# louissmit/VBNN

Measured on AMD Instinct MI355X. Metric: VBLinear fwd+bwd samples/sec, higher is better.
Workload: dtype bf16; 1 GPU; 784-4096-4096-10 VBLinear MLP, batch 4096 per GPU, LRT, S=1; mode=lrt, global_batch=4096, parallelism=dp1, warmup_steps_run=255, backward_order=every updateGradInput, then the accGradParameters from the first layer up, launch=one stream launch per kernel

## Files before the change

### vbnn_amd/csrc/elementwise.hip

```cpp
#include "common.h"

static inline int grid_for(int64_t work_items, int per_block) {
    int64_t b = (work_items + per_block - 1) / per_block;
    if (b < 1) b = 1;
    if (b > 2048) b = 2048;
    return (int)b;
}

template <bool HW>
__global__ __launch_bounds__(256) void k_fill_normal(float* out, int64_t rows, int64_t cols, int64_t ld, uint64_t seed,
                                                     uint32_t stream, uint32_t layer, uint32_t draw, int64_t row0, float scale) {
    const int64_t quads = (cols + 3) >> 2;
    const int64_t total = rows * quads;
    for (int64_t t = (int64_t)blockIdx.x * 256 + threadIdx.x; t < total; t += (int64_t)gridDim.x * 256) {
        const int64_t r = t / quads, q = t - r * quads;
        const vbnn_f32x4 z = HW ? vbnn_normal4_hw(seed, stream, layer, draw, (uint32_t)(row0 + r), (uint32_t)q)
                                : vbnn_normal4(seed, stream, layer, draw, (uint32_t)(row0 + r), (uint32_t)q);
        float* p = out + r * ld + q * 4;
        const int valid = (int)min((int64_t)4, cols - q * 4);
        const bool vec = ((ld & 3) == 0) && (((uintptr_t)out & 15u) == 0);
        store4<float>(p, z.v[0] * scale, z.v[1] * scale, z.v[2] * scale, z.v[3] * scale, valid, vec);
    }
}

// ... 1010 lines not shown
        else hipLaunchKernelGGL(k_update_finish<bf16_t>, dim3(n_layers + pack_blocks), dim3(256), 0, ctx->stream, fa);
    }
    return vbnn_check_launch("vbnn_update");
    VBNN_API_END
}

template <typename T>
__global__ __launch_bounds__(256) void k_pack_input(const float* __restrict__ src, int64_t ld_src, int64_t N, int64_t I, T* x_s,
                                                    T* x2_s, int64_t ld_x, T* xT_s, T* x2T_s, int64_t ld_xT, int64_t rpd) {
    __shared__ float ta[64][65];
    __shared__ float tb[64][65];
    const int64_t tiles_c = (I + 63) / 64, tiles_r = (N + 63) / 64;
    const int64_t ntiles = tiles_c * tiles_r;
    const bool vec_in = ((ld_src & 3) == 0) && (((uintptr_t)src & 15u) == 0);
    const bool vec_t = (ld_xT & 3) == 0;
    for (int64_t tI = blockIdx.x; tI < ntiles; tI += gridDim.x) {
        const int64_t r0 = (tI / tiles_c) * 64, c0 = (tI % tiles_c) * 64;
#pragma unroll
        for (int k = 0; k < 4; ++k) {
            const int idx = threadIdx.x + 256 * k;
            const int rr = idx >> 4, c4 = (idx & 15) * 4;
            const int64_t r = r0 + rr, c = c0 + c4;
            float a[4] = {0.f, 0.f, 0.f, 0.f}, b[4] = {0.f, 0.f, 0.f, 0.f};
            const int valid = (r < N) ? (int)min((int64_t)4, I - c) : 0;
            if (valid > 0) {
                load4<float>(src + (rpd > 0 ? r % rpd : r) * ld_src + c, a, valid, vec_in);
#pragma unroll
                for (int e = 0; e < 4; ++e) { const float ar = Elt<T>::from(Elt<T>::to(a[e])); b[e] = ar * ar; }
                store4<T>(x_s + r * ld_x + c, a[0], a[1], a[2], a[3], valid, true);
                if (x2_s) store4<T>(x2_s + r * ld_x + c, b[0], b[1], b[2], b[3], valid, true);
            }
#pragma unroll
            for (int e = 0; e < 4; ++e) { ta[rr][c4 + e] = a[e]; tb[rr][c4 + e] = b[e]; }
        }
        if (xT_s) {
            __syncthreads();
#pragma unroll
            for (int k = 0; k < 4; ++k) {
                const int idx = threadIdx.x + 256 * k;
                const int cc = idx >> 4, r4 = (idx & 15) * 4;
                const int64_t c = c0 + cc, r = r0 + r4;
                const int valid = (c < I) ? (int)min((int64_t)4, N - r) : 0;
                if (valid > 0) {
                    store4<T>(xT_s + c * ld_xT + r, ta[r4][cc], ta[r4 + 1][cc], ta[r4 + 2][cc], ta[r4 + 3][cc], valid, vec_t);
                    if (x2T_s)
                        store4<T>(x2T_s + c * ld_xT + r, tb[r4][cc], tb[r4 + 1][cc], tb[r4 + 2][cc], tb[r4 + 3][cc], valid, vec_t);
                }
            }
            __syncthreads();
        }
    }
}

extern "C" int vbnn_pack_input(vbnn_ctx* ctx, int dtype, const float* src, int64_t ld_src, int64_t N, int64_t I, void* x_s,
                               void* x2_s, int64_t ld_x, void* xT_s, void* x2T_s, int64_t ld_xT, int64_t rows_per_draw) {
    VBNN_API_BEGIN
    VBNN_REQUIRE(ctx && src && x_s, "null argument");
    VBNN_REQUIRE(rows_per_draw >= 0, "rows_per_draw");
    VBNN_REQUIRE(N > 0 && I > 0 && ld_src >= I && ld_x >= I && ld_x % 4 == 0, "shape");
    VBNN_REQUIRE(!x2T_s || xT_s, "x2T_s needs xT_s");
    VBNN_REQUIRE(!xT_s || ld_xT >= N, "ld_xT");
    const int64_t ntiles = ((N + 63) / 64) * ((I + 63) / 64);
    const int nb = (int)(ntiles < 4096 ? ntiles : 4096);
    if (dtype == VBNN_F32)
        hipLaunchKernelGGL(k_pack_input<float>, dim3(nb), dim3(256), 0, ctx->stream, src, ld_src, N, I, (float*)x_s, (float*)x2_s,
                           ld_x, (float*)xT_s, (float*)x2T_s, ld_xT, rows_per_draw);
    else if (dtype == VBNN_BF16)
        hipLaunchKernelGGL(k_pack_input<bf16_t>, dim3(nb), dim3(256), 0, ctx->stream, src, ld_src, N, I, (bf16_t*)x_s,
                           (bf16_t*)x2_s, ld_x, (bf16_t*)xT_s, (bf16_t*)x2T_s, ld_xT, rows_per_draw);
    else { vbnn_set_error("unsupported dtype %d", dtype); return VBNN_ERR_UNSUPPORTED; }
    return vbnn_check_launch("k_pack_input");
    VBNN_API_END
}

template <bool TO_BF16>
__global__ __launch_bounds__(256) void k_cast_grads(const void* __restrict__ src, void* __restrict__ dst, int64_t n, int vec) {
    const int64_t i0 = ((int64_t)blockIdx.x * 256 + threadIdx.x) * 8;
    if (i0 >= n) return;
    if (vec && i0 + 8 <= n) {
        if constexpr (TO_BF16) {
            const f32x4 a = reinterpret_cast<const f32x4*>(static_cast<const float*>(src) + i0)[0];
            const f32x4 b = reinterpret_cast<const f32x4*>(static_cast<const float*>(src) + i0)[1];
            reinterpret_cast<bf16x8*>(static_cast<bf16_t*>(dst) + i0)[0] =
                bf16x8{(bf16_t)a[0], (bf16_t)a[1], (bf16_t)a[2], (bf16_t)a[3], (bf16_t)b[0], (bf16_t)b[1], (bf16_t)b[2], (bf16_t)b[3]};
        } else {
            const bf16x8 v = reinterpret_cast<const bf16x8*>(static_cast<const bf16_t*>(src) + i0)[0];
            reinterpret_cast<f32x4*>(static_cast<float*>(dst) + i0)[0] = f32x4{(float)v[0], (float)v[1], (float)v[2], (float)v[3]};
            reinterpret_cast<f32x4*>(static_cast<float*>(dst) + i0)[1] = f32x4{(float)v[4], (float)v[5], (float)v[6], (float)v[7]};
        }
    } else {
        for (int64_t i = i0; i < n && i < i0 + 8; ++i) {
            if constexpr (TO_BF16) static_cast<bf16_t*>(dst)[i] = (bf16_t)static_cast<const float*>(src)[i];
            else static_cast<float*>(dst)[i] = (float)static_cast<const bf16_t*>(src)[i];
        }
    }
}

extern "C" int vbnn_cast_grads(vbnn_ctx* ctx, int to_bf16, const void* src, void* dst, int64_t n) {
    VBNN_API_BEGIN
    VBNN_REQUIRE(ctx && src && dst && n > 0, "argument");
    const int vec = (((uintptr_t)src | (uintptr_t)dst) & 15u) == 0;
    const unsigned nb = (unsigned)((n + 2047) / 2048);
    if (to_bf16) hipLaunchKernelGGL(k_cast_grads<true>, dim3(nb), dim3(256), 0, ctx->stream, src, dst, n, vec);
    else hipLaunchKernelGGL(k_cast_grads<false>, dim3(nb), dim3(256), 0, ctx->stream, src, dst, n, vec);
    return vbnn_check_launch("k_cast_grads");
    VBNN_API_END
}

struct StatsCombineArgs { double* stats[8]; int n_layers, world; const double* parts; };
__global__ void k_stats_combine(StatsCombineArgs a) {
    const int l = threadIdx.x;
    if (l >= a.n_layers) return;
    double s0 = 0.0, s1 = 0.0, w = 0.0;
    for (int r = 0; r < a.world; ++r) {
// ... 47 lines not shown
```

### vbnn_amd/csrc/head.hip

```cpp
#include "common.h"
#include "gemm_v1.h"

constexpr int HEAD_CMAX = 16;
constexpr int HEAD_FW = 8;

template <typename T> struct Vec8;
template <> struct Vec8<bf16_t> {
    typedef bf16x8 raw_t;
    static __device__ __forceinline__ raw_t load_raw(const bf16_t* p) { return *reinterpret_cast<const bf16x8*>(p); }
    static __device__ __forceinline__ void cvt(const raw_t& t, float (&v)[8]) {
#pragma unroll
        for (int e = 0; e < 8; ++e) v[e] = (float)t[e];
    }
    static __device__ __forceinline__ raw_t load_guarded(const bf16_t* p, int valid) {
        raw_t t;
#pragma unroll
        for (int e = 0; e < 8; ++e) t[e] = e < valid ? p[e] : (bf16_t)0.f;
        return t;
    }
    static __device__ __forceinline__ void load(const bf16_t* p, float (&v)[8]) {
        const bf16x8 t = *reinterpret_cast<const bf16x8*>(p);
#pragma unroll
        for (int e = 0; e < 8; ++e) v[e] = (float)t[e];
    }
// ... 28 lines not shown
        *reinterpret_cast<f32x4*>(p) = f32x4{v[0], v[1], v[2], v[3]};
        *reinterpret_cast<f32x4*>(p + 4) = f32x4{v[4], v[5], v[6], v[7]};
    }
};

__device__ __forceinline__ float head_sum_partials(const float* src, int64_t stride, int R) {
    float tot = 0.f;
    int r = 0;
    for (; r + 8 <= R; r += 8) {
        float p[8];
#pragma unroll
        for (int u = 0; u < 8; ++u) p[u] = vbnn_load_wt(src + (int64_t)(r + u) * stride);
#pragma unroll
        for (int u = 0; u < 8; ++u) tot += p[u];
    }
    if (r < R) {
        float p[8];
#pragma unroll
        for (int u = 0; u < 8; ++u) p[u] = (r + u < R) ? vbnn_load_wt(src + (int64_t)(r + u) * stride) : 0.f;
#pragma unroll
        for (int u = 0; u < 8; ++u) if (r + u < R) tot += p[u];
    }
    return tot;
}

__device__ __forceinline__ void head_row_max(const float (&v)[4], int q, float& mx, int& arg) {
    mx = -INFINITY; arg = 0x7fffffff;
#pragma unroll
    for (int j = 0; j < 4; ++j)
        if (v[j] > mx) { mx = v[j]; arg = 4 * q + j; }
#pragma unroll
    for (int off = 16; off <= 32; off <<= 1) {
        const float om = __shfl_xor(mx, off, 64);
        const int oa = __shfl_xor(arg, off, 64);
        if (om > mx || (om == mx && oa < arg)) { mx = om; arg = oa; }
    }
}

__device__ __forceinline__ void head_log_softmax(f32x4 s, int q, int C, const float* __restrict__ bias, float (&lg)[4], int& arg, float& lse) {
#pragma unroll
    for (int j = 0; j < 4; ++j) {
        const int c = 4 * q + j;
        lg[j] = (c < C) ? s[j] + (bias ? bias[c] : 0.f) : -INFINITY;
    }
    float mx;
    head_row_max(lg, q, mx, arg);
    float se = 0.f;
#pragma unroll
    for (int j = 0; j < 4; ++j) if (4 * q + j < C) se += expf(lg[j] - mx);
    se += __shfl_xor(se, 16, 64);
    se += __shfl_xor(se, 32, 64);
    lse = mx + logf(se);
}

__device__ __forceinline__ void head_rows_from_logits(f32x4 s, int lane, int64_t n0, int64_t N, int C, const float* __restrict__ bias,
                                                      const int32_t* __restrict__ target, int64_t rpd, float inv_n, float* out, float* g_logits,
                                                      float* logits, double* part_loss, int32_t* part_corr) {
    const int q = lane >> 4, c16 = lane & 15;
    const int64_t n = n0 + c16;
    const bool row_ok = n < N;
    float lg[4];
    int arg;
    float lse;
    head_log_softmax(s, q, C, bias, lg, arg, lse);
    const int t = row_ok ? min(max(target[rpd > 0 ? n % rpd : n], 0), C - 1) : 0;
    double loss_acc = 0.0;
#pragma unroll
    for (int j = 0; j < 4; ++j) {
        const int c = 4 * q + j;
        if (row_ok && c < C) {
            const float o = lg[j] - lse;
            if (logits) logits[n * C + c] = lg[j];
            if (out) out[n * C + c] = o;
            g_logits[n * C + c] = (expf(o) - (c == t ? 1.0f : 0.0f)) * inv_n;
            if (c == t) loss_acc -= (double)o * (double)inv_n;
        }
    }
    int corr = (row_ok && q == 0 && arg == t) ? 1 : 0;
#pragma unroll
    for (int off = 32; off > 0; off >>= 1) { loss_acc += __shfl_xor(loss_acc, off, 64); corr += __shfl_xor(corr, off, 64); }
    if (lane == 0) { vbnn_store_wt(&part_loss[blockIdx.x], loss_acc); vbnn_store_wt(&part_corr[blockIdx.x], (int32_t)corr); }
}

template <int NT>
__device__ __forceinline__ void head_sum_loss_partials(unsigned* counter, const double* part_loss, const int32_t* part_corr, double* loss_sum,
                                                       int32_t* correct, int accumulate, double* red_l, int* red_c, int* last) {
    if (!vbnn_last_arriver(counter, gridDim.x, last)) return;
    const int lane = threadIdx.x & 63, wave = threadIdx.x >> 6;
    double ls = 0.0;
    int cs = 0;
    for (int b = (int)threadIdx.x; b < (int)gridDim.x; b += NT) { ls += vbnn_load_wt(&part_loss[b]); cs += vbnn_load_wt(&part_corr[b]); }
#pragma unroll
    for (int off = 32; off > 0; off >>= 1) { ls += __shfl_xor(ls, off, 64); cs += __shfl_xor(cs, off, 64); }
    if (lane == 0) { red_l[wave] = ls; red_c[wave] = cs; }
    __syncthreads();
    if (threadIdx.x == 0) {
        double lt = 0.0;
        int ct = 0;
#pragma unroll
        for (int w = 0; w < NT / 64; ++w) { lt += red_l[w]; ct += red_c[w]; }
        if (loss_sum) loss_sum[0] = (accumulate ? loss_sum[0] : 0.0) + lt;
        if (correct) correct[0] = (accumulate ? correct[0] : 0) + ct;
    }
}

template <typename T>
__device__ __forceinline__ f32x4 head_logits_wave(const T* __restrict__ hp, const T* __restrict__ wp, int64_t k_lo, int64_t k_hi) {
// ... 458 lines not shown
        }
    }
    auto put = [&](float* p, float v) { if (fin_tickets) vbnn_store_wt(p, v); else *p = v; };
    if (partial_w) {
        const int64_t i = c0 + 16 * wave + c16;
        if (i < H) {
#pragma unroll
            for (int j = 0; j < 4; ++j)
                if (4 * q + j < C) put(&partial_w[((int64_t)blockIdx.y * C + 4 * q + j) * H + i], accw[j]);
            if (partial_bp && q == 0) put(&partial_bp[(int64_t)blockIdx.y * H + i], accp[0]);
        }
    }
    if (partial_b && blockIdx.x == 0) {
        __syncthreads();
        float* red = reinterpret_cast<float*>(&th[0][0]);
        red[tid] = accb;
        __syncthreads();
        if (tid < C) {
            float tot = 0.f;
#pragma unroll
            for (int rg = 0; rg < 16; ++rg) tot += red[rg * 16 + tid];
            put(&partial_b[(int64_t)blockIdx.y * C + tid], tot);
        }
    }
    if (!fin_tickets) return;
    __shared__ int fin_last;
    if (!vbnn_last_arriver(fin_tickets + blockIdx.x, gridDim.y, &fin_last)) return;
    const int R = (int)gridDim.y;
    const int64_t nw = (int64_t)C * H;
    for (int k = tid; k < C * 64 + 64; k += 256) {
        const bool is_w = k < C * 64;
        const int64_t i = c0 + (is_w ? k & 63 : k - C * 64);
        if (i >= H) continue;
        float* dst = is_w ? (fin_gw ? fin_gw + (int64_t)(k >> 6) * H + i : nullptr) : (fin_gbp ? fin_gbp + i : nullptr);
        if (!dst) continue;
        const float* src = is_w ? partial_w + (int64_t)(k >> 6) * H + i : partial_bp + i;
        const int64_t stride = is_w ? nw : H;
        const float tot = head_sum_partials(src, stride, R);
        *dst = (fin_accumulate ? *dst : 0.f) + tot;
    }
    if (blockIdx.x == 0 && tid < C && fin_gb) {
        const float tot = head_sum_partials(partial_b + tid, C, R);
        fin_gb[tid] = (fin_accumulate ? fin_gb[tid] : 0.f) + tot;
    }
}

typedef __bf16 hb_bf16x2 __attribute__((ext_vector_type(2)));
__device__ __forceinline__ float hb_dot2(unsigned a, unsigned b, float c) {
    return __builtin_amdgcn_fdot2_f32_bf16(__builtin_bit_cast(hb_bf16x2, a), __builtin_bit_cast(hb_bf16x2, b), c, false);
}
__device__ __forceinline__ unsigned hb_bf16_bits(float v) {
    return (unsigned)__builtin_bit_cast(unsigned short, (bf16_t)v);
}
template <int U, int HEAD_SW >
__global__ __launch_bounds__(64 * HEAD_SW) void k_head_backward_stream(
    const bf16_t* __restrict__ h, int64_t ld_h, const bf16_t* __restrict__ w3, int64_t ld_w, const float* __restrict__ g, int64_t N,
    int64_t H, int C, int relu_mask, const bf16_t* __restrict__ r_prev, int64_t ld_r, bf16_t* __restrict__ g_prev,
    bf16_t* __restrict__ gv_prev, int64_t ld_gp, int rows_per_chunk, float* __restrict__ partial_w ,
    float* __restrict__ partial_b , float* __restrict__ partial_bp ,
    unsigned* fin_tickets , int fin_accumulate, float* fin_gw, float* fin_gb, float* fin_gbp) {
    static_assert(U == 2 || U == 4, "2 or 4 hidden units per lane");
    constexpr int CP = 12, NP = CP / 2, UW = U / 2;
    typedef float accv __attribute__((ext_vector_type(U)));
    typedef unsigned rawv __attribute__((ext_vector_type(UW)));
    __shared__ accv red[4][HEAD_SW][64];
    const int tid = threadIdx.x, lane = tid & 63, wave = tid >> 6;
    const int64_t cb0 = (int64_t)blockIdx.x * (64 * U);
    const int64_t c0 = cb0 + U * lane;
    const int64_t n_lo = (int64_t)blockIdx.y * rows_per_chunk, n_hi = min(N, n_lo + rows_per_chunk);
    unsigned wp[NP][U];
    {
        unsigned wr[CP][UW];
#pragma unroll
        for (int c = 0; c < CP; ++c) {
            rawv t = 0u;
            if (c < C) t = *reinterpret_cast<const rawv*>(w3 + (int64_t)c * ld_w + c0);
#pragma unroll
            for (int k = 0; k < UW; ++k) wr[c][k] = ((const unsigned*)&t)[k];
        }
#pragma unroll
        for (int p = 0; p < NP; ++p)
#pragma unroll
            for (int e = 0; e < U; ++e) {
                const unsigned lo = (wr[2 * p][e >> 1] >> (16 * (e & 1))) & 0xffffu, hi = (wr[2 * p + 1][e >> 1] >> (16 * (e & 1))) & 0xffffu;
                wp[p][e] = lo | (hi << 16);
            }
    }
    float accw[CP][U], accb[U], accg = 0.f;
#pragma unroll
    for (int e = 0; e < U; ++e) accb[e] = 0.f;
#pragma unroll
    for (int c = 0; c < CP; ++c)
#pragma unroll
        for (int e = 0; e < U; ++e) accw[c][e] = 0.f;
    const int gcls = lane < CP ? lane : lane - CP;
    const bool gl_on = lane < 2 * CP && gcls < C;
    const bool has_r = r_prev != nullptr;
    const unsigned lo_h = (unsigned)(U * lane);
    auto ldrow = [&](int64_t n, rawv& hv, rawv& rv) {
        hv = *reinterpret_cast<const rawv*>(h + (n * ld_h + cb0) + lo_h);
        rv = 0u;
        if (has_r) rv = *reinterpret_cast<const rawv*>(r_prev + (n * ld_r + cb0) + lo_h);
    };
    auto ldg = [&](int64_t n) { return gl_on ? g[(n + (lane >= CP ? 1 : 0)) * C + gcls] : 0.f; };
    auto word = [](const rawv& v, int k) { return ((const unsigned*)&v)[k]; };
    int64_t n = n_lo + 2 * wave;
    rawv h0 = 0u, h1 = 0u, r0 = 0u, r1 = 0u;
    float gv = 0.f;
    if (n < n_hi) { ldrow(n, h0, r0); ldrow(n + 1, h1, r1); gv = ldg(n); }
    for (; n < n_hi; n += 2 * HEAD_SW) {
        const rawv hh[2] = {h0, h1}, rr[2] = {r0, r1};
        const float cg = gv;
        const int64_t nn = n + 2 * HEAD_SW;
        if (nn < n_hi) { ldrow(nn, h0, r0); ldrow(nn + 1, h1, r1); gv = ldg(nn); }
        accg += cg;
        const unsigned gb = hb_bf16_bits(cg);
        unsigned g0[CP], g1[CP];
#pragma unroll
        for (int c = 0; c < CP; ++c) { g0[c] = __builtin_amdgcn_readlane(gb, c); g1[c] = __builtin_amdgcn_readlane(gb, CP + c); }
#pragma unroll
        for (int row = 0; row < 2; ++row) {
            const unsigned* gs = row ? g1 : g0;
            float gx[U];
#pragma unroll
            for (int e = 0; e < U; ++e) gx[e] = 0.f;
#pragma unroll
            for (int p = 0; p < NP; ++p) {
                const unsigned gp2 = gs[2 * p] | (gs[2 * p + 1] << 16);
#pragma unroll
                for (int e = 0; e < U; ++e) gx[e] = hb_dot2(gp2, wp[p][e], gx[e]);
            }
            unsigned gbits[U], vbits[U];
#pragma unroll
            for (int e = 0; e < U; ++e) {
                const unsigned hw = word(hh[row], e >> 1), rw = word(rr[row], e >> 1);
                const float hv = __builtin_bit_cast(float, (e & 1) ? (hw & 0xffff0000u) : (hw << 16));
                const float rv = __builtin_bit_cast(float, (e & 1) ? (rw & 0xffff0000u) : (rw << 16));
                const float gp = (relu_mask && !(hv > 0.f)) ? 0.f : gx[e];
                gbits[e] = hb_bf16_bits(gp);
                vbits[e] = hb_bf16_bits(has_r ? gp * rv : 0.f);
                accb[e] += __builtin_bit_cast(float, gbits[e] << 16);
            }
            const int64_t ro = (n + row) * ld_gp + cb0;
            rawv og, ov;
#pragma unroll
            for (int k = 0; k < UW; ++k) { ((unsigned*)&og)[k] = gbits[2 * k] | (gbits[2 * k + 1] << 16); ((unsigned*)&ov)[k] = vbits[2 * k] | (vbits[2 * k + 1] << 16); }
            *reinterpret_cast<rawv*>(g_prev + ro + lo_h) = og;
            if (gv_prev) *reinterpret_cast<rawv*>(gv_prev + ro + lo_h) = ov;
        }
        unsigned hp[U];
#pragma unroll
        for (int e = 0; e < U; ++e) {
            const unsigned a = word(hh[0], e >> 1), b = word(hh[1], e >> 1);
            hp[e] = (e & 1) ? ((a >> 16) | (b & 0xffff0000u)) : ((a & 0xffffu) | (b << 16));
        }
#pragma unroll
        for (int c = 0; c < CP; ++c) {
            const unsigned gr2 = g0[c] | (g1[c] << 16);
#pragma unroll
            for (int e = 0; e < U; ++e) accw[c][e] = hb_dot2(gr2, hp[e], accw[c][e]);
        }
    }
    const int64_t chunk = blockIdx.y;
    auto put = [&](float* p, const accv& t) {
        if (!fin_tickets) { *reinterpret_cast<accv*>(p) = t; return; }
#pragma unroll
        for (int e = 0; e < U; e += 2) vbnn_store_wt2(p + e, t[e], t[e + 1]);
    };
    auto meet = [&](const accv (&q)[4], int nq, auto&& emit) {
        __syncthreads();
#pragma unroll
        for (int k = 0; k < 4; ++k)
            if (k < nq) red[k][wave][lane] = q[k];
        __syncthreads();
        if (wave < nq) {
            accv t = red[wave][0][lane];
#pragma unroll
            for (int w = 1; w < HEAD_SW; ++w) t += red[wave][w][lane];
            emit(wave, t);
        }
    };
#pragma unroll
    for (int c4 = 0; c4 < CP; c4 += 4) {
        accv q[4];
#pragma unroll
        for (int k = 0; k < 4; ++k)
#pragma unroll
            for (int e = 0; e < U; ++e) q[k][e] = accw[c4 + k][e];
        meet(q, 4, [&](int k, accv t) {
            if (partial_w && c4 + k < C) put(partial_w + ((chunk * C + c4 + k) * H + c0), t);
        });
    }
    {
        accv q[4];
#pragma unroll
        for (int k = 0; k < 4; ++k)
#pragma unroll
            for (int e = 0; e < U; ++e) q[k][e] = (k == 0) ? accb[e] : ((k == 1 && e == 0) ? accg : 0.f);
        meet(q, 2, [&](int k, accv t) {
            const float odd = __shfl(t[0], (lane + CP) & 63, 64);
            if (k == 0) { if (partial_bp) put(partial_bp + (chunk * H + c0), t); }
            else if (partial_b && blockIdx.x == 0 && lane < CP && lane < C) {
                if (fin_tickets) vbnn_store_wt(&partial_b[chunk * C + lane], t[0] + odd); else partial_b[chunk * C + lane] = t[0] + odd;
            }
        });
    }
    if (!fin_tickets) return;
    __shared__ int fin_last;
    if (!vbnn_last_arriver(fin_tickets + blockIdx.x, gridDim.y, &fin_last)) return;
    const int R = (int)gridDim.y;
    const int64_t nw = (int64_t)C * H;
    constexpr int CB = 64 * U;
    for (int k = tid; k < C * CB + CB; k += 64 * HEAD_SW) {
// ... 276 lines not shown
                                       int64_t N, int64_t C, float inv_n, float* logits, float* out, float* g_logits, int accumulate,
                                       double* loss_sum_dev, int32_t* correct_dev, int64_t rows_per_draw) {
    VBNN_API_BEGIN
    VBNN_REQUIRE(ctx && slots && target && g_logits, "null argument");
    VBNN_REQUIRE(rows_per_draw >= 0, "rows_per_draw");
    VBNN_REQUIRE(N > 0 && C > 0 && C <= HEAD_CMAX && n_slots > 0 && n_slots < (1 << 20), "shape (C <= 16)");
    VBNN_REQUIRE(((uintptr_t)slots & 15u) == 0, "slots must be 16-byte aligned");
    const unsigned nb = (unsigned)((N + 15) / 16);
    VBNN_REQUIRE((size_t)nb * 2 <= ctx->scratch_doubles, "minibatch too large for the reduction scratch");
    double* part_loss = ctx->scratch;
    int32_t* part_corr = reinterpret_cast<int32_t*>(ctx->scratch + nb);
    hipLaunchKernelGGL(k_head_from_slots, dim3(nb), dim3(64), 0, ctx->stream, slots, (int)n_slots, bias, target, N, (int)C, inv_n, out,
                       g_logits, logits, loss_sum_dev, correct_dev, accumulate, part_loss, part_corr, ctx->counters + VBNN_CNT_HEAD_FWD,
                       rows_per_draw);
    return vbnn_check_launch("k_head_from_slots");
    VBNN_API_END
}

extern "C" int vbnn_head_predict(vbnn_ctx* ctx, int dtype, const vbnn_predict_args* a) {
    VBNN_API_BEGIN
    VBNN_REQUIRE(ctx && a && a->h && a->w3, "null argument");
    VBNN_REQUIRE(a->R > 0 && a->H > 0 && a->C > 0 && a->C <= HEAD_CMAX, "shape (C <= 16)");
    VBNN_REQUIRE(a->S >= 1 && a->S < (1ll << 24), "draws S >= 1");
    VBNN_REQUIRE(a->form == VBNN_PREDICT_STACKED || a->form == VBNN_PREDICT_ACCUMULATE, "form");
    VBNN_REQUIRE(a->ld_h % VBNN_KPAD == 0 && a->ld_w % VBNN_KPAD == 0 && a->ld_h >= a->H && a->ld_w >= a->H, "h and w3 must be packed operands");
    VBNN_REQUIRE((((uintptr_t)a->h | (uintptr_t)a->w3) & 15u) == 0, "operands must be 16-byte aligned");
    VBNN_REQUIRE(!a->totals || a->target, "totals need targets");
    const bool stacked = a->form == VBNN_PREDICT_STACKED;
    const int draws = stacked ? (int)a->S : 1;
    const int first = stacked ? 1 : (a->first ? 1 : 0), fin = stacked ? 1 : (a->final ? 1 : 0);
    VBNN_REQUIRE(a->state || (first && fin), "the accumulating form keeps its running state in `state`");
    VBNN_REQUIRE(a->R * draws < (1ll << 40), "rows");
    const unsigned nb = (unsigned)((a->R + 15) / 16);
    VBNN_REQUIRE((size_t)nb * 4 <= ctx->scratch_doubles, "minibatch too large for the reduction scratch");
    double* part = ctx->scratch;
    unsigned* ticket = ctx->counters + VBNN_CNT_PREDICT;
    if (dtype == VBNN_F32) {
        const int64_t Hp = (a->H + 15) / 16 * 16;
        hipLaunchKernelGGL(k_head_predict<float>, dim3(nb), dim3(64 * HEAD_FW), 0, ctx->stream, (const float*)a->h, a->ld_h,
                           (const float*)a->w3, a->ld_w, a->bias, a->target, a->R, Hp, (int)a->C, draws, (int)a->S, first, fin,
                           a->state, a->probs, a->log_probs, a->entropy, a->expected_entropy, a->mutual_info, a->pred, a->totals,
                           part, ticket);
    } else if (dtype == VBNN_BF16) {
        const int64_t Hp = (a->H + 31) / 32 * 32;
        hipLaunchKernelGGL(k_head_predict<bf16_t>, dim3(nb), dim3(64 * HEAD_FW), 0, ctx->stream, (const bf16_t*)a->h, a->ld_h,
                           (const bf16_t*)a->w3, a->ld_w, a->bias, a->target, a->R, Hp, (int)a->C, draws, (int)a->S, first, fin,
                           a->state, a->probs, a->log_probs, a->entropy, a->expected_entropy, a->mutual_info, a->pred, a->totals,
                           part, ticket);
    } else { vbnn_set_error("unsupported dtype %d", dtype); return VBNN_ERR_UNSUPPORTED; }
    return vbnn_check_launch("k_head_predict");
    VBNN_API_END
}

static int g_head_inline_finish = 1;
template <typename T>
static int head_backward_t(vbnn_ctx* ctx, const T* h, int64_t ld_h, const T* w3, int64_t ld_w, const float* g_logits, int64_t N,
                           int64_t H, int64_t C, int accumulate, float* gradWeight, float* gradBias, float* gradBias_prev,
                           int relu_mask, const void* r_prev_any, int64_t ld_r_prev, int r_prev_packed, T* g_prev, T* gv_prev,
                           int64_t ld_gp, T* gT_prev, T* gvT_prev, int64_t ld_gpT) {
    const float* r_prev = r_prev_packed ? nullptr : (const float*)r_prev_any;
    const T* r_prev_t = r_prev_packed ? (const T*)r_prev_any : nullptr;
    const bool sums = gradWeight || gradBias || gradBias_prev;
    if (!sums && !g_prev && !gT_prev) return VBNN_OK;
    static const bool env_read = [] { const char* e = getenv("VBNN_HEAD_INLINE_FINISH"); if (e && e[0] == '0') g_head_inline_finish = 0; return true; }();
    (void)env_read;
    const int64_t tiles_c = (H + 63) / 64, tiles_r = (N + 63) / 64;
    const int64_t per_chunk = C * H + C + H;
    const int64_t cap = (int64_t)(ctx->scratch_doubles * 2) / per_chunk;
    VBNN_REQUIRE(!sums || cap >= 1, "hidden size too large for the reduction scratch");
    int64_t R = (2 * (int64_t)vbnn_cu_count() + tiles_c - 1) / tiles_c;
    static const int env_blocks = [] { const char* e = getenv("VBNN_HEAD_BLOCKS"); return e ? atoi(e) : 0; }();
    if (env_blocks > 0) R = (env_blocks + tiles_c - 1) / tiles_c;
    if (R > tiles_r) R = tiles_r;
    if (sums && R > cap) R = cap;
    if (R < 1) R = 1;
    VBNN_REQUIRE(R <= 65535, "too many row chunks");
    const int rows_per_chunk = (int)((tiles_r + R - 1) / R) * 64;
    R = (N + rows_per_chunk - 1) / rows_per_chunk;
    float* partial_w = reinterpret_cast<float*>(ctx->scratch);
    float* partial_b = partial_w + R * C * H;
    float* partial_bp = partial_b + R * C;
    const bool vec = (ld_h % 8 == 0) && (!r_prev_any || ld_r_prev % 8 == 0) && (!g_prev || ld_gp % 8 == 0) &&
                     (!(gT_prev || gvT_prev) || ld_gpT % 8 == 0) &&
                     ((((uintptr_t)h | (uintptr_t)r_prev_any | (uintptr_t)g_prev | (uintptr_t)gv_prev | (uintptr_t)gT_prev |
                        (uintptr_t)gvT_prev) & 15u) == 0);
    const dim3 grid((unsigned)tiles_c, (unsigned)R);
    float* pw = (gradWeight || gradBias_prev) ? partial_w : nullptr;
    float* pb = gradBias ? partial_b : nullptr;
    float* pbp = gradBias_prev ? partial_bp : nullptr;
    const bool full = vec && (H % 64 == 0) && (N % 64 == 0) && N * ld_h < (1ll << 31) && N * ld_gp < (1ll << 31) &&
                      H * ld_gpT < (1ll << 31) && (!r_prev_any || N * ld_r_prev < (1ll << 31));
    const bool inline_fin = sums && tiles_c * R <= vbnn_cu_count() && tiles_c <= VBNN_CNT_TILES_MAX && g_head_inline_finish;
    unsigned* ft = inline_fin ? ctx->counters + VBNN_CNT_TILES : nullptr;
    static const bool env_stream = [] { const char* e = getenv("VBNN_HEAD_STREAM"); return !(e && e[0] == '0'); }();
    if constexpr (sizeof(T) == 2) {
        const bool want = g_head_stream == 1 || (g_head_stream == -1 && env_stream && !inline_fin);
        if (want && full && C <= 12 && !r_prev && g_prev && !gT_prev && !gvT_prev && H % 128 == 0 && N % 32 == 0) {
            constexpr int SU = 2, SWV = 16;
            if (H % (64 * SU) == 0 && N % (2 * SWV) == 0) {
            const int64_t cb = H / (64 * SU);
            int64_t Rs = ((int64_t)vbnn_cu_count() + cb - 1) / cb;
            if (Rs < 1) Rs = 1;
            if (sums && Rs > cap) Rs = cap;
            const int rpc = (int)(((N + Rs - 1) / Rs + 2 * SWV - 1) / (2 * SWV) * (2 * SWV));
            Rs = (N + rpc - 1) / rpc;
            float* spw = reinterpret_cast<float*>(ctx->scratch);
            float* spb = spw + Rs * C * H;
            float* spbp = spb + Rs * C;
#define VBNN_HS_LAUNCH(UU, WW) hipLaunchKernelGGL((k_head_backward_stream<UU, WW>), dim3((unsigned)cb, (unsigned)Rs), dim3(64 * WW), 0, ctx->stream, (const bf16_t*)h, ld_h, \
                               (const bf16_t*)w3, ld_w, g_logits, N, H, (int)C, relu_mask, (const bf16_t*)r_prev_t, ld_r_prev, (bf16_t*)g_prev,  \
                               (bf16_t*)gv_prev, ld_gp, rpc, (gradWeight || gradBias_prev) ? spw : nullptr, gradBias ? spb : nullptr,         \
                               gradBias_prev ? spbp : nullptr, sft, accumulate, gradWeight, gradBias, gradBias_prev)
            unsigned* sft = (sums && g_head_inline_finish && cb <= VBNN_CNT_TILES_MAX) ? ctx->counters + VBNN_CNT_TILES : nullptr;
            VBNN_HS_LAUNCH(SU, SWV);
#undef VBNN_HS_LAUNCH
            if (sums && !sft) {
                const int64_t outs = C * H + (gradBias_prev ? H : 0);
                hipLaunchKernelGGL(k_head_backward_finish, dim3((unsigned)((outs + 255) / 256)), dim3(256), 0, ctx->stream, spw, spb, spbp,
                                   (int)Rs, H, (int)C, accumulate, gradWeight, gradBias, gradBias_prev);
            }
            return vbnn_check_launch("k_head_backward_stream");
            }
        }
    }
    if (full && C <= 12 && !r_prev)
        hipLaunchKernelGGL((k_head_backward<T, true, true, 12>), grid, dim3(256), 0, ctx->stream, h, ld_h, w3, ld_w, g_logits, N, H, (int)C,
                           relu_mask, r_prev, r_prev_t, ld_r_prev, g_prev, gv_prev, ld_gp, gT_prev, gvT_prev, ld_gpT, rows_per_chunk,
                           pw, pb, pbp, ft, accumulate, gradWeight, gradBias, gradBias_prev);
    else if (full)
        hipLaunchKernelGGL((k_head_backward<T, true, true>), grid, dim3(256), 0, ctx->stream, h, ld_h, w3, ld_w, g_logits, N, H, (int)C,
                           relu_mask, r_prev, r_prev_t, ld_r_prev, g_prev, gv_prev, ld_gp, gT_prev, gvT_prev, ld_gpT, rows_per_chunk,
                           pw, pb, pbp, ft, accumulate, gradWeight, gradBias, gradBias_prev);
    else if (vec)
        hipLaunchKernelGGL((k_head_backward<T, true, false>), grid, dim3(256), 0, ctx->stream, h, ld_h, w3, ld_w, g_logits, N, H, (int)C,
                           relu_mask, r_prev, r_prev_t, ld_r_prev, g_prev, gv_prev, ld_gp, gT_prev, gvT_prev, ld_gpT, rows_per_chunk,
                           pw, pb, pbp, ft, accumulate, gradWeight, gradBias, gradBias_prev);
    else
        hipLaunchKernelGGL((k_head_backward<T, false, false>), grid, dim3(256), 0, ctx->stream, h, ld_h, w3, ld_w, g_logits, N, H, (int)C,
                           relu_mask, r_prev, r_prev_t, ld_r_prev, g_prev, gv_prev, ld_gp, gT_prev, gvT_prev, ld_gpT, rows_per_chunk,
                           pw, pb, pbp, ft, accumulate, gradWeight, gradBias, gradBias_prev);
    if (sums && !inline_fin) {
        const int64_t outs = C * H + (gradBias_prev ? H : 0);
        hipLaunchKernelGGL(k_head_backward_finish, dim3((unsigned)((outs + 255) / 256)), dim3(256), 0, ctx->stream, partial_w,
                           partial_b, partial_bp, (int)R, H, (int)C, accumulate, gradWeight, gradBias, gradBias_prev);
    }
    return vbnn_check_launch("k_head_backward");
}

extern "C" int vbnn_head_backward(vbnn_ctx* ctx, int dtype, const void* h, int64_t ld_h, const void* w3, int64_t ld_w,
                                  const float* g_logits, int64_t N, int64_t H, int64_t C, int accumulate, float* gradWeight,
                                  float* gradBias, float* gradBias_prev, int relu_mask, const void* r_prev, int64_t ld_r_prev,
                                  int r_prev_packed, void* g_prev, void* gv_prev, int64_t ld_gp, void* gT_prev, void* gvT_prev,
                                  int64_t ld_gpT) {
    VBNN_API_BEGIN
    VBNN_REQUIRE(ctx && h && w3 && g_logits, "null argument");
    vbnn_cu_scope plan(ctx);
    VBNN_REQUIRE(N > 0 && H > 0 && C > 0 && C <= HEAD_CMAX, "shape (C <= 16)");
    VBNN_REQUIRE(ld_h % VBNN_KPAD == 0 && ld_h >= H && ld_w >= H, "h and w3 must be packed operands");
    VBNN_REQUIRE(!gv_prev || (g_prev && r_prev), "gv_prev needs g_prev and r_prev");
    VBNN_REQUIRE(!(g_prev || gv_prev) || ld_gp >= H, "ld_gp");
    VBNN_REQUIRE(!(gT_prev || gvT_prev) || ld_gpT >= N, "ld_gpT");
    if (dtype == VBNN_F32)
        return head_backward_t<float>(ctx, (const float*)h, ld_h, (const float*)w3, ld_w, g_logits, N, H, C, accumulate, gradWeight,
                                      gradBias, gradBias_prev, relu_mask, r_prev, ld_r_prev, r_prev_packed, (float*)g_prev, (float*)gv_prev,
                                      ld_gp, (float*)gT_prev, (float*)gvT_prev, ld_gpT);
    if (dtype == VBNN_BF16)
        return head_backward_t<bf16_t>(ctx, (const bf16_t*)h, ld_h, (const bf16_t*)w3, ld_w, g_logits, N, H, C, accumulate,
                                       gradWeight, gradBias, gradBias_prev, relu_mask, r_prev, ld_r_prev, r_prev_packed, (bf16_t*)g_prev,
// ... 52 lines not shown
```

Before: 5.455 million samples/s.

## Deepen head backward stream prefetch and add flat input pack kernel

The streaming head-backward kernel now keeps a configurable number of row pairs in flight (default two), using a register ring buffer and sched barriers so loads are issued well ahead of the dot-product work. The r_prev/gv_prev path becomes a compile-time flag, and the wave index is made uniform with readfirstlane. Separately, input packing gets a flat vectorized elementwise kernel for the case where no transposed copy is needed, replacing the tiled transpose kernel there. The deeper prefetch raises register pressure and could lower occupancy.

```diff
diff --git a/vbnn_amd/csrc/elementwise.hip b/vbnn_amd/csrc/elementwise.hip
--- a/vbnn_amd/csrc/elementwise.hip
+++ b/vbnn_amd/csrc/elementwise.hip
@@ -1086,6 +1086,47 @@
     }
 }
 
+template <typename T>
+__global__ __launch_bounds__(256) void k_pack_input_flat(const float* __restrict__ src, int64_t ld_src, int64_t N, int64_t I,
+                                                         T* __restrict__ x_s, T* __restrict__ x2_s, int64_t ld_x, int64_t rpd, int vec_in,
+                                                         int vec_out) {
+    const unsigned octs = (unsigned)((I + 7) >> 3);
+    const unsigned total = (unsigned)N * octs;
+    for (unsigned t = blockIdx.x * 256u + threadIdx.x; t < total; t += gridDim.x * 256u) {
+        const unsigned r = t / octs, c = (t - r * octs) * 8u;
+        const int64_t sr = rpd > 0 ? (int64_t)r % rpd : (int64_t)r;
+        const float* sp = src + sr * ld_src + c;
+        const int valid = (int)min((int64_t)8, I - c);
+        float a[8], b[8];
+        if (vec_in && valid == 8) {
+            const f32x4 lo = reinterpret_cast<const f32x4*>(sp)[0], hi = reinterpret_cast<const f32x4*>(sp)[1];
+#pragma unroll
+            for (int e = 0; e < 4; ++e) { a[e] = lo[e]; a[4 + e] = hi[e]; }
+        } else {
+#pragma unroll
+            for (int e = 0; e < 8; ++e) a[e] = e < valid ? sp[e] : 0.f;
+        }
+#pragma unroll
+        for (int e = 0; e < 8; ++e) { const float ar = Elt<T>::from(Elt<T>::to(a[e])); b[e] = ar * ar; }
+        T* xp = x_s + (int64_t)r * ld_x + c;
+        T* x2p = x2_s ? x2_s + (int64_t)r * ld_x + c : nullptr;
+        if (vec_out && valid == 8) {
+            if constexpr (sizeof(T) == 2) {
+                *reinterpret_cast<bf16x8*>(xp) = bf16x8{(bf16_t)a[0], (bf16_t)a[1], (bf16_t)a[2], (bf16_t)a[3], (bf16_t)a[4], (bf16_t)a[5], (bf16_t)a[6], (bf16_t)a[7]};
+                if (x2p) *reinterpret_cast<bf16x8*>(x2p) = bf16x8{(bf16_t)b[0], (bf16_t)b[1], (bf16_t)b[2], (bf16_t)b[3], (bf16_t)b[4], (bf16_t)b[5], (bf16_t)b[6], (bf16_t)b[7]};
+            } else {
+                reinterpret_cast<f32x4*>(xp)[0] = f32x4{a[0], a[1], a[2], a[3]};
+                reinterpret_cast<f32x4*>(xp)[1] = f32x4{a[4], a[5], a[6], a[7]};
+                if (x2p) { reinterpret_cast<f32x4*>(x2p)[0] = f32x4{b[0], b[1], b[2], b[3]}; reinterpret_cast<f32x4*>(x2p)[1] = f32x4{b[4], b[5], b[6], b[7]}; }
+            }
+        } else {
+#pragma unroll
+            for (int e = 0; e < 8; ++e)
+                if (e < valid) { xp[e] = Elt<T>::to(a[e]); if (x2p) x2p[e] = Elt<T>::to(b[e]); }
+        }
+    }
+}
+
 extern "C" int vbnn_pack_input(vbnn_ctx* ctx, int dtype, const float* src, int64_t ld_src, int64_t N, int64_t I, void* x_s,
                                void* x2_s, int64_t ld_x, void* xT_s, void* x2T_s, int64_t ld_xT, int64_t rows_per_draw) {
     VBNN_API_BEGIN
@@ -1094,6 +1135,19 @@
     VBNN_REQUIRE(N > 0 && I > 0 && ld_src >= I && ld_x >= I && ld_x % 4 == 0, "shape");
     VBNN_REQUIRE(!x2T_s || xT_s, "x2T_s needs xT_s");
     VBNN_REQUIRE(!xT_s || ld_xT >= N, "ld_xT");
+    const int64_t octs = N * ((I + 7) / 8);
+    if (!xT_s && octs < (1ll << 31) && (dtype == VBNN_F32 || dtype == VBNN_BF16)) {
+        const int vec_in = (ld_src % 4 == 0) && (((uintptr_t)src & 15u) == 0);
+        const int vec_out = (ld_x % (dtype == VBNN_BF16 ? 8 : 4) == 0) && ((((uintptr_t)x_s | (uintptr_t)x2_s) & 15u) == 0);
+        const int nb = grid_for(octs, 256);
+        if (dtype == VBNN_F32)
+            hipLaunchKernelGGL(k_pack_input_flat<float>, dim3(nb), dim3(256), 0, ctx->stream, src, ld_src, N, I, (float*)x_s, (float*)x2_s,
+                               ld_x, rows_per_draw, vec_in, vec_out);
+        else
+            hipLaunchKernelGGL(k_pack_input_flat<bf16_t>, dim3(nb), dim3(256), 0, ctx->stream, src, ld_src, N, I, (bf16_t*)x_s,
+                               (bf16_t*)x2_s, ld_x, rows_per_draw, vec_in, vec_out);
+        return vbnn_check_launch("k_pack_input_flat");
+    }
     const int64_t ntiles = ((N + 63) / 64) * ((I + 63) / 64);
     const int nb = (int)(ntiles < 4096 ? ntiles : 4096);
     if (dtype == VBNN_F32)
diff --git a/vbnn_amd/csrc/head.hip b/vbnn_amd/csrc/head.hip
--- a/vbnn_amd/csrc/head.hip
+++ b/vbnn_amd/csrc/head.hip
@@ -104,7 +104,6 @@
     se += __shfl_xor(se, 32, 64);
     lse = mx + logf(se);
 }
-
 __device__ __forceinline__ void head_rows_from_logits(f32x4 s, int lane, int64_t n0, int64_t N, int C, const float* __restrict__ bias,
                                                       const int32_t* __restrict__ target, int64_t rpd, float inv_n, float* out, float* g_logits,
                                                       float* logits, double* part_loss, int32_t* part_corr) {
@@ -669,7 +668,7 @@
 __device__ __forceinline__ unsigned hb_bf16_bits(float v) {
     return (unsigned)__builtin_bit_cast(unsigned short, (bf16_t)v);
 }
-template <int U, int HEAD_SW >
+template <int U, int HEAD_SW , int AHEAD, bool HAS_V>
 __global__ __launch_bounds__(64 * HEAD_SW) void k_head_backward_stream(
     const bf16_t* __restrict__ h, int64_t ld_h, const bf16_t* __restrict__ w3, int64_t ld_w, const float* __restrict__ g, int64_t N,
     int64_t H, int C, int relu_mask, const bf16_t* __restrict__ r_prev, int64_t ld_r, bf16_t* __restrict__ g_prev,
@@ -677,11 +676,13 @@
     float* __restrict__ partial_b , float* __restrict__ partial_bp ,
     unsigned* fin_tickets , int fin_accumulate, float* fin_gw, float* fin_gb, float* fin_gbp) {
     static_assert(U == 2 || U == 4, "2 or 4 hidden units per lane");
+    static_assert(AHEAD >= 1 && AHEAD <= 4, "row pairs in flight");
     constexpr int CP = 12, NP = CP / 2, UW = U / 2;
     typedef float accv __attribute__((ext_vector_type(U)));
     typedef unsigned rawv __attribute__((ext_vector_type(UW)));
     __shared__ accv red[4][HEAD_SW][64];
-    const int tid = threadIdx.x, lane = tid & 63, wave = tid >> 6;
+    const int tid = threadIdx.x, lane = tid & 63;
+    const int wave = __builtin_amdgcn_readfirstlane(tid >> 6);
     const int64_t cb0 = (int64_t)blockIdx.x * (64 * U);
     const int64_t c0 = cb0 + U * lane;
     const int64_t n_lo = (int64_t)blockIdx.y * rows_per_chunk, n_hi = min(N, n_lo + rows_per_chunk);
@@ -712,70 +713,89 @@
         for (int e = 0; e < U; ++e) accw[c][e] = 0.f;
     const int gcls = lane < CP ? lane : lane - CP;
     const bool gl_on = lane < 2 * CP && gcls < C;
-    const bool has_r = r_prev != nullptr;
     const unsigned lo_h = (unsigned)(U * lane);
     auto ldrow = [&](int64_t n, rawv& hv, rawv& rv) {
         hv = *reinterpret_cast<const rawv*>(h + (n * ld_h + cb0) + lo_h);
         rv = 0u;
-        if (has_r) rv = *reinterpret_cast<const rawv*>(r_prev + (n * ld_r + cb0) + lo_h);
+        if constexpr (HAS_V) rv = *reinterpret_cast<const rawv*>(r_prev + (n * ld_r + cb0) + lo_h);
     };
-    auto ldg = [&](int64_t n) { return gl_on ? g[(n + (lane >= CP ? 1 : 0)) * C + gcls] : 0.f; };
+    const int g_off = lane < 2 * CP ? (lane >= CP ? C : 0) + min(gcls, C - 1) : 0;
+    auto ldg = [&](int64_t n) { return g[n * C + g_off]; };
     auto word = [](const rawv& v, int k) { return ((const unsigned*)&v)[k]; };
+    constexpr int64_t STEP = 2 * HEAD_SW;
+    rawv hq[AHEAD][2], rq[AHEAD][2];
+    float gq[AHEAD];
+    auto ldstage = [&](int s, int64_t nn) { ldrow(nn, hq[s][0], rq[s][0]); ldrow(nn + 1, hq[s][1], rq[s][1]); gq[s] = ldg(nn); };
     int64_t n = n_lo + 2 * wave;
-    rawv h0 = 0u, h1 = 0u, r0 = 0u, r1 = 0u;
-    float gv = 0.f;
-    if (n < n_hi) { ldrow(n, h0, r0); ldrow(n + 1, h1, r1); gv = ldg(n); }
-    for (; n < n_hi; n += 2 * HEAD_SW) {
-        const rawv hh[2] = {h0, h1}, rr[2] = {r0, r1};
-        const float cg = gv;
-        const int64_t nn = n + 2 * HEAD_SW;
-        if (nn < n_hi) { ldrow(nn, h0, r0); ldrow(nn + 1, h1, r1); gv = ldg(nn); }
-        accg += cg;
-        const unsigned gb = hb_bf16_bits(cg);
-        unsigned g0[CP], g1[CP];
-#pragma unroll
-        for (int c = 0; c < CP; ++c) { g0[c] = __builtin_amdgcn_readlane(gb, c); g1[c] = __builtin_amdgcn_readlane(gb, CP + c); }
-#pragma unroll
-        for (int row = 0; row < 2; ++row) {
-            const unsigned* gs = row ? g1 : g0;
-            float gx[U];
-#pragma unroll
-            for (int e = 0; e < U; ++e) gx[e] = 0.f;
-#pragma unroll
-            for (int p = 0; p < NP; ++p) {
-                const unsigned gp2 = gs[2 * p] | (gs[2 * p + 1] << 16);
-#pragma unroll
-                for (int e = 0; e < U; ++e) gx[e] = hb_dot2(gp2, wp[p][e], gx[e]);
-            }
-            unsigned gbits[U], vbits[U];
+#pragma unroll
+    for (int s = 0; s < AHEAD; ++s) {
+        hq[s][0] = hq[s][1] = rq[s][0] = rq[s][1] = 0u; gq[s] = 0.f;
+        if (n + s * STEP < n_hi) ldstage(s, n + s * STEP);
+    }
+    auto pair = [&](int s, int64_t n, bool more) {
+            const rawv hh[2] = {hq[s][0], hq[s][1]}, rr[2] = {rq[s][0], rq[s][1]};
+            const float cg = gl_on ? gq[s] : 0.f;
+            __builtin_amdgcn_sched_barrier(0);
+            if (more) ldstage(s, n + AHEAD * STEP);
+            __builtin_amdgcn_sched_barrier(0);
+            accg += cg;
+            const unsigned gb = hb_bf16_bits(cg);
+            unsigned g0[CP], g1[CP];
+#pragma unroll
+            for (int c = 0; c < CP; ++c) { g0[c] = __builtin_amdgcn_readlane(gb, c); g1[c] = __builtin_amdgcn_readlane(gb, CP + c); }
+#pragma unroll
+            for (int row = 0; row < 2; ++row) {
+                const unsigned* gs = row ? g1 : g0;
+                float gx[U];
+#pragma unroll
+                for (int e = 0; e < U; ++e) gx[e] = 0.f;
+#pragma unroll
+                for (int p = 0; p < NP; ++p) {
+                    const unsigned gp2 = gs[2 * p] | (gs[2 * p + 1] << 16);
+#pragma unroll
+                    for (int e = 0; e < U; ++e) gx[e] = hb_dot2(gp2, wp[p][e], gx[e]);
+                }
+                unsigned gbits[U], vbits[U];
+#pragma unroll
+                for (int e = 0; e < U; ++e) {
+                    const unsigned hw = word(hh[row], e >> 1), rw = word(rr[row], e >> 1);
+                    const float hv = __builtin_bit_cast(float, (e & 1) ? (hw & 0xffff0000u) : (hw << 16));
+                    const float rv = __builtin_bit_cast(float, (e & 1) ? (rw & 0xffff0000u) : (rw << 16));
+                    const float gp = (relu_mask && !(hv > 0.f)) ? 0.f : gx[e];
+                    gbits[e] = hb_bf16_bits(gp);
+                    vbits[e] = hb_bf16_bits(HAS_V ? gp * rv : 0.f);
+                    accb[e] += __builtin_bit_cast(float, gbits[e] << 16);
+                }
+                const int64_t ro = (n + row) * ld_gp + cb0;
+                rawv og, ov;
+#pragma unroll
+                for (int k = 0; k < UW; ++k) { ((unsigned*)&og)[k] = gbits[2 * k] | (gbits[2 * k + 1] << 16); ((unsigned*)&ov)[k] = vbits[2 * k] | (vbits[2 * k + 1] << 16); }
+                *reinterpret_cast<rawv*>(g_prev + ro + lo_h) = og;
+                if constexpr (HAS_V) *reinterpret_cast<rawv*>(gv_prev + ro + lo_h) = ov;
+            }
+            unsigned hp[U];
 #pragma unroll
             for (int e = 0; e < U; ++e) {
-                const unsigned hw = word(hh[row], e >> 1), rw = word(rr[row], e >> 1);
-                const float hv = __builtin_bit_cast(float, (e & 1) ? (hw & 0xffff0000u) : (hw << 16));
-                const float rv = __builtin_bit_cast(float, (e & 1) ? (rw & 0xffff0000u) : (rw << 16));
-                const float gp = (relu_mask && !(hv > 0.f)) ? 0.f : gx[e];
-                gbits[e] = hb_bf16_bits(gp);
-                vbits[e] = hb_bf16_bits(has_r ? gp * rv : 0.f);
-                accb[e] += __builtin_bit_cast(float, gbits[e] << 16);
-            }
-            const int64_t ro = (n + row) * ld_gp + cb0;
-            rawv og, ov;
-#pragma unroll
-            for (int k = 0; k < UW; ++k) { ((unsigned*)&og)[k] = gbits[2 * k] | (gbits[2 * k + 1] << 16); ((unsigned*)&ov)[k] = vbits[2 * k] | (vbits[2 * k + 1] << 16); }
-            *reinterpret_cast<rawv*>(g_prev + ro + lo_h) = og;
-            if (gv_prev) *reinterpret_cast<rawv*>(gv_prev + ro + lo_h) = ov;
-        }
-        unsigned hp[U];
-#pragma unroll
-        for (int e = 0; e < U; ++e) {
-            const unsigned a = word(hh[0], e >> 1), b = word(hh[1], e >> 1);
-            hp[e] = (e & 1) ? ((a >> 16) | (b & 0xffff0000u)) : ((a & 0xffffu) | (b << 16));
-        }
-#pragma unroll
-        for (int c = 0; c < CP; ++c) {
-            const unsigned gr2 = g0[c] | (g1[c] << 16);
-#pragma unroll
-            for (int e = 0; e < U; ++e) accw[c][e] = hb_dot2(gr2, hp[e], accw[c][e]);
+                const unsigned a = word(hh[0], e >> 1), b = word(hh[1], e >> 1);
+                hp[e] = (e & 1) ? ((a >> 16) | (b & 0xffff0000u)) : ((a & 0xffffu) | (b << 16));
+            }
+#pragma unroll
+            for (int c = 0; c < CP; ++c) {
+                const unsigned gr2 = g0[c] | (g1[c] << 16);
+#pragma unroll
+                for (int e = 0; e < U; ++e) accw[c][e] = hb_dot2(gr2, hp[e], accw[c][e]);
+            }
+    };
+    for (; n + (2 * AHEAD - 1) * STEP < n_hi; n += AHEAD * STEP) {
+#pragma unroll
+        for (int s = 0; s < AHEAD; ++s) pair(s, n + s * STEP, true);
+    }
+    for (; n < n_hi; n += AHEAD * STEP) {
+#pragma unroll
+        for (int s = 0; s < AHEAD; ++s) {
+            const int64_t nc = n + s * STEP;
+            if (nc >= n_hi) break;
+            pair(s, nc, nc + AHEAD * STEP < n_hi);
         }
     }
     const int64_t chunk = blockIdx.y;
@@ -1158,6 +1178,7 @@
     VBNN_API_END
 }
 
+#define VBNN_HEAD_AHEAD_DEFAULT 2
 static int g_head_inline_finish = 1;
 template <typename T>
 static int head_backward_t(vbnn_ctx* ctx, const T* h, int64_t ld_h, const T* w3, int64_t ld_w, const float* g_logits, int64_t N,
@@ -1202,7 +1223,9 @@
     if constexpr (sizeof(T) == 2) {
         const bool want = g_head_stream == 1 || (g_head_stream == -1 && env_stream && !inline_fin);
         if (want && full && C <= 12 && !r_prev && g_prev && !gT_prev && !gvT_prev && H % 128 == 0 && N % 32 == 0) {
+            static const int env_ahead = [] { const char* e = getenv("VBNN_HEAD_AHEAD"); return e ? atoi(e) : 0; }();
             constexpr int SU = 2, SWV = 16;
+            const int ahead = env_ahead >= 1 && env_ahead <= 2 ? env_ahead : VBNN_HEAD_AHEAD_DEFAULT;
             if (H % (64 * SU) == 0 && N % (2 * SWV) == 0) {
             const int64_t cb = H / (64 * SU);
             int64_t Rs = ((int64_t)vbnn_cu_count() + cb - 1) / cb;
@@ -1213,13 +1236,15 @@
             float* spw = reinterpret_cast<float*>(ctx->scratch);
             float* spb = spw + Rs * C * H;
             float* spbp = spb + Rs * C;
-#define VBNN_HS_LAUNCH(UU, WW) hipLaunchKernelGGL((k_head_backward_stream<UU, WW>), dim3((unsigned)cb, (unsigned)Rs), dim3(64 * WW), 0, ctx->stream, (const bf16_t*)h, ld_h, \
+#define VBNN_HS_LAUNCH1(UU, WW, AA, VV) hipLaunchKernelGGL((k_head_backward_stream<UU, WW, AA, VV>), dim3((unsigned)cb, (unsigned)Rs), dim3(64 * WW), 0, ctx->stream, (const bf16_t*)h, ld_h, \
                                (const bf16_t*)w3, ld_w, g_logits, N, H, (int)C, relu_mask, (const bf16_t*)r_prev_t, ld_r_prev, (bf16_t*)g_prev,  \
                                (bf16_t*)gv_prev, ld_gp, rpc, (gradWeight || gradBias_prev) ? spw : nullptr, gradBias ? spb : nullptr,         \
                                gradBias_prev ? spbp : nullptr, sft, accumulate, gradWeight, gradBias, gradBias_prev)
             unsigned* sft = (sums && g_head_inline_finish && cb <= VBNN_CNT_TILES_MAX) ? ctx->counters + VBNN_CNT_TILES : nullptr;
-            VBNN_HS_LAUNCH(SU, SWV);
+#define VBNN_HS_LAUNCH(AA) do { if (gv_prev) VBNN_HS_LAUNCH1(SU, SWV, AA, true); else VBNN_HS_LAUNCH1(SU, SWV, AA, false); } while (0)
+            if (ahead == 1) VBNN_HS_LAUNCH(1); else VBNN_HS_LAUNCH(2);
 #undef VBNN_HS_LAUNCH
+#undef VBNN_HS_LAUNCH1
             if (sums && !sft) {
                 const int64_t outs = C * H + (gradBias_prev ? H : 0);
                 hipLaunchKernelGGL(k_head_backward_finish, dim3((unsigned)((outs + 255) / 256)), dim3(256), 0, ctx->stream, spw, spb, spbp,
```

After: 5.480 million samples/s (median of 2 runs). No clear change (+0.5%).
